# spacejam/tla-rust

Hardware: AMD Instinct MI355X
Metric: distinct states/sec, raft.tla (3 servers) (higher is better)
Workload: dtype u64

## Files before the change

### tla_rust_amd/csrc/engine.hip

```cpp
#include <hip/hip_runtime.h>
#include <hipcub/hipcub.hpp>

#include <algorithm>
#include <chrono>
#include <memory>
#include <type_traits>
#include <string>
#include <vector>

#include "spec_registry.h"
#include "hip_owned.h"

namespace mc {

#ifndef MC_TU
#define MC_TU -1
#endif
}
extern "C" void mc_set_error_internal(const char *msg);
namespace mc {
static void set_error(const std::string &s) { mc_set_error_internal(s.c_str()); }

#define HIP_TRY(expr)                                                                              \
    do {                                                                                           \
// ... 21 lines not shown
    double progress_interval = 1.0;
    std::chrono::steady_clock::time_point progress_last;
    bool stop_requested = false;
    void report_progress(uint32_t levels, uint64_t generated, uint64_t distinct, uint64_t queue) {
        if (!progress_fn) return;
        const auto now = std::chrono::steady_clock::now();
        if (std::chrono::duration<double>(now - progress_last).count() < progress_interval) return;
        progress_last = now;
        progress_fn(progress_user, levels, generated, distinct, queue);
    }
    virtual ~EngineBase() = default;
    virtual int run(mc_result *out) = 0;
    virtual int step(uint32_t levels, mc_result *out) = 0;
    virtual int trace(uint8_t *states_out, int32_t *actions_out, size_t *n_inout) = 0;
    virtual int kernel_stats(mc_kernel_stats *out) = 0;
    virtual int read_states(uint64_t first, uint64_t count, uint8_t *out) = 0;
    virtual int debug_reexpand(unsigned extra_flags, double *ms) = 0;
    virtual int debug_phases(uint64_t *out48, int reset) = 0;
    virtual int debug_flags(uint32_t set, uint32_t clear) = 0;
    virtual int checkpoint(const char *path) = 0;
    virtual int restore(const char *path) = 0;
    virtual int shard_begin() = 0;
    virtual int shard_begin_replicated(uint64_t min_frontier, uint64_t max_distinct, uint64_t max_levels, uint64_t *levels_out, uint32_t *nlevels) = 0;
    virtual int shard_level_size(uint64_t *n) = 0;
    virtual int shard_set_stream(void *hip_stream, int enable) = 0;
    virtual int shard_expand_launch(unsigned slot, uint64_t first, uint64_t count, uint64_t send_cap) = 0;
    virtual int shard_expand_finish(unsigned slot, uint64_t *send_fp, uint64_t send_cap, uint64_t *send_counts) = 0;
    virtual int shard_probe(const uint64_t *recv_fp, uint64_t n, uint8_t *answers) = 0;
    virtual int shard_expand_pack(unsigned slot, uint64_t *send_fp, uint64_t cap) = 0;
    virtual int shard_probe_pack(const uint64_t *recv_fp, uint64_t cap, uint8_t *answers) = 0;
    virtual int shard_keep_pack(unsigned slot, const uint8_t *answers_back, uint64_t cap) = 0;
    virtual int shard_wait_keep(unsigned slot) = 0;
    virtual int shard_materialise(unsigned slot, const uint8_t *answers_back, uint8_t *send_states, uint64_t send_cap, uint64_t *send_counts) = 0;
    virtual int shard_ingest(const uint8_t *recv_states, uint64_t n) = 0;
    virtual int shard_keep(unsigned slot, const uint8_t *answers_back, uint64_t *n_new) = 0;
    virtual int shard_end_level(uint64_t *new_local) = 0;
    virtual int shard_counters(uint64_t *generated, uint64_t *distinct_local, int32_t *verdict) = 0;
    virtual int shard_check_frontier() = 0;
    virtual int shard_materialise_parents(unsigned slot, uint64_t *send_parents) = 0;
    virtual int shard_ingest_parents(const uint64_t *recv_parents, uint64_t n, unsigned src_rank) = 0;
    virtual int shard_violation(int32_t *found, uint64_t *idx, uint32_t *slot, int32_t *verdict, int32_t *invariant) = 0;
    virtual int shard_fetch(uint64_t idx, uint8_t *state_out, uint32_t *parent_rank, uint64_t *parent_idx, uint32_t *parent_slot) = 0;
    virtual int shard_info(void **main_stream, uint64_t *chunk_states, int32_t *traced) = 0;
    virtual int shard_note_levels(const uint64_t *levels, uint32_t n, int32_t verdict) = 0;
    virtual int shard_resume(uint64_t *levels_out, uint32_t *nlevels) = 0;
    virtual int shard_checkpoint(const char *path) = 0;
    virtual int shard_restore(const char *path) = 0;
    virtual size_t state_bytes() const = 0;
    virtual int simulate(const mc_sim_opts *opts, mc_sim_result *out) = 0;
    virtual int coverage(mc_action_coverage *out, size_t *n_inout) = 0;
    virtual int graph(mc_graph_info *out) = 0;
    virtual int graph_read(uint64_t first, uint64_t count, uint64_t *offsets_out, uint32_t *dst_out, int32_t *action_out, size_t *nedges_inout) = 0;
    virtual int scc(mc_scc_info *out) = 0;
    virtual int scc_read(uint64_t first, uint64_t count, uint32_t *scc_out) = 0;
    virtual int liveness(uint64_t weak_fair_mask, mc_live_info *out) = 0;
    virtual int liveness_trace(uint32_t *prefix_out, size_t *nprefix_inout, uint32_t *cycle_out, size_t *ncycle_inout) = 0;
};

static uint64_t round_pow2(uint64_t v) {
    uint64_t p = 1;
    while (p < v) p <<= 1;
    return p;
}

struct KTimer {
    std::vector<Event> pool;
    struct Pending { int which; size_t e0, e1; uint64_t units; };
    std::vector<Pending> pending;
    size_t used = 0;
    bool enabled = false;
    hipEvent_t get() {
        if (used == pool.size()) pool.emplace_back(hipEventDefault);
        return pool[used++].get();
    }
    void resolve(mc_kernel_stat *stats ) {
        for (auto &p : pending) {
            float ms = 0;
            hipEventElapsedTime(&ms, pool[p.e0].get(), pool[p.e1].get());
            stats[p.which].launches++;
            stats[p.which].ms_total += ms;
            stats[p.which].units += p.units;
        }
        pending.clear();
        used = 0;
    }
};

template <class S, class = void>
struct HasExport : std::false_type {};
template <class S>
struct HasExport<S, decltype((void)S::EXPORT_WORDS)> : std::true_type {};
template <class S, class = void>
struct PackedRows : std::false_type {};
template <class S>
struct PackedRows<S, decltype((void)S::PACKED_ROWS)> : std::integral_constant<bool, S::PACKED_ROWS> {};

static_assert((unsigned)SIM_VK_INVARIANT == VK_INVARIANT && (unsigned)SIM_VK_ASSERT == VK_ASSERT && (unsigned)SIM_VK_DEADLOCK == VK_DEADLOCK, "one verdict_of_kind");
static int32_t verdict_of_kind(unsigned kind) {
    return kind == VK_INVARIANT ? MC_V_INVARIANT : kind == VK_ASSERT ? MC_V_ASSERT : kind == VK_DEADLOCK ? MC_V_DEADLOCK : MC_V_SPECERR;
}
struct Viol {
    unsigned kind, slot;
    int32_t verdict, invariant;
    explicit Viol(unsigned long long key)
        : kind((unsigned)(key & 7u)), slot((unsigned)(key >> 8 & 0xffffu)), verdict(verdict_of_kind(kind)), invariant(kind == VK_INVARIANT ? (int32_t)(key >> 3 & 31u) : -1) {}
    bool extra_state() const { return kind == VK_INVARIANT && slot < SLOT_PARENT; }
};

struct CkIdent {
    char magic[8];
    uint32_t spec_id, nparams;
    int64_t params[16];
    uint32_t words, has_trace;
};
struct CkHeader {
    CkIdent id;
    uint64_t distinct, generated, cells, lo, hi, nlevels;
};
struct ShCkHeader {
    CkIdent id;
    uint32_t rank, world;
    uint64_t table_cap, lo, hi, next, dup, nlevels;
};
struct ShCkCounters {
    uint64_t arena_next, viol_key, via_list;
    uint64_t generated[NSHARD], cells[NSHARD];
    uint32_t error, pad;
};
static_assert(sizeof(CkIdent) == 152 && offsetof(CkIdent, spec_id) == 8 && offsetof(CkIdent, params) == 16 && offsetof(CkIdent, words) == 144 && offsetof(CkIdent, has_trace) == 148, "checkpoint identity");
static_assert(sizeof(CkHeader) == 200 && offsetof(CkHeader, distinct) == 152 && offsetof(CkHeader, generated) == 160 && offsetof(CkHeader, cells) == 168 &&
              offsetof(CkHeader, lo) == 176 && offsetof(CkHeader, hi) == 184 && offsetof(CkHeader, nlevels) == 192, "TLAMCCK1 header");
static_assert(sizeof(ShCkHeader) == 208 && offsetof(ShCkHeader, rank) == 152 && offsetof(ShCkHeader, world) == 156 && offsetof(ShCkHeader, table_cap) == 160 &&
              offsetof(ShCkHeader, lo) == 168 && offsetof(ShCkHeader, hi) == 176 && offsetof(ShCkHeader, next) == 184 && offsetof(ShCkHeader, dup) == 192 &&
              offsetof(ShCkHeader, nlevels) == 200, "TLAMCSK2 header");
static_assert(NSHARD == 8 && sizeof(ShCkCounters) == 160 && offsetof(ShCkCounters, generated) == 24 && offsetof(ShCkCounters, cells) == 88 && offsetof(ShCkCounters, error) == 152, "TLAMCSK2 counters");
struct CkFormat { const char *magic, *writer, *reader, *not_ours, *other_program; };
static constexpr CkFormat CK_FUSED{"TLAMCCK1", "checkpoint", "restore", "not a checkpoint file",
                                   "the checkpoint was written by another compiled program (algorithm, constants, invariants or constraints differ)"};
static constexpr CkFormat CK_RANK{"TLAMCSK2", "mc_shard_checkpoint", "mc_shard_restore", "not a per-rank checkpoint file (of this library version)",
                                  "the checkpoint was written by another compiled program"};
struct CkPart { void *p; size_t bytes; };
struct FileCloser { FILE *f; ~FileCloser() { if (f) fclose(f); } };

template <class S>
struct Engine : EngineBase {
    using Params = typename S::Params;
    int W = 1;
    unsigned max_slots = 1;
    Params prm;
    mc_spec_desc desc;
    mc_config cfg;
    Stream stream, stream2;
    Stream stream_b;
    Event ev_level, ev_e[2], ev_m[2];
    DevBuf<uint64_t> d_arena, d_table, d_cand, d_inittmp;
    DevBuf<uint32_t> d_newlist, d_parent;
    DevBuf<uint64_t> d_newfp;
    DevBuf<uint16_t> d_nsl, d_pslot;
    DevBuf<uint8_t> d_prank;
    DevBuf<DevCounters> d_ctr;
    PinnedBuf<DevCounters> h_ctr;
    DevBuf<LevelCtl> d_lc;
    PinnedBuf<LevelCtl> h_lc;
    uint64_t table_cap = 0, arena_cap = 0, chunk = 0, row_stride = 0, seg_cap = 0;
    bool seen_sparse = false, use_matrix = false;
    bool no_slices = getenv("TLAMC_NOSLICE") != nullptr;
    double inwave_growth_limit = getenv("TLAMC_INWAVE_GROWTH") ? atof(getenv("TLAMC_INWAVE_GROWTH")) : 10.0;
    KTimer timer;
    mc_kernel_stat kstat[3];
    struct Fused {
        bool have_run = false, have_viol = false;
        unsigned long long last_viol = ~0ull;
        std::vector<uint64_t> level_start;
        uint64_t last_distinct = 0, last_generated = 0, cells = 0, inwave = 0;
        uint64_t stop_frontier = 0, lo = 0, hi = 0;
        bool mat_inwave_level = false;
        uint64_t mat_list_hint = 0;
    } fr;
    struct HandOver {
        bool pending = false, in_place = false;
        uint64_t distinct = 0, generated = 0, cells = 0, lo = 0;
        std::vector<uint64_t> level_start;
    } ck;
    struct ShSlot {
        DevBuf<uint64_t> rt_fp;
        DevBuf<uint32_t> rt_src, pend_src;
        DevBuf<PaddedCounter> rt_cur;
        uint64_t rt_subcap = 0, pend_total = 0, chunk_base = 0, count = 0, ncols = 0;
        BlockPlan plan;
        uint64_t moved = 0;
        OwnerOffsets pend_off;
        bool launched = false, keep_pending = false;
    };
    struct Shard {
        uint64_t lo = 0, hi = 0, next = 0;
        uint64_t dup = 0;
        ShSlot sl[2];
        DevBuf<uint32_t> d_new_src, d_incl;
        DevBuf<unsigned long long> d_ends;
        PinnedBuf<unsigned long long> h_ends;
        PinnedBuf<PaddedCounter> h_cur;
        DevBuf<char> d_scan_tmp;
        hipStream_t ext_stream = nullptr;
        bool ext_side = false;
        Event ev_slot[2], ev_keep[2], ev_ans;
        Event ev_append;
        Event ev_exp[2];
        Event ev_mat[2];
        std::vector<uint64_t> levels;
        bool ck_ok = false, resume = false;
        std::unique_ptr<mc_result> prefix_res{new mc_result()};
    } sh;
    struct Sim {
        DevBuf<uint64_t> buf[2];
        DevBuf<uint32_t> wst;
        DevBuf<SimCounters> ctr;
        std::vector<uint64_t> trace_rows;
        std::vector<int32_t> trace_acts;
        size_t trace_n = 0;
    } sim;
    struct Cov {
        bool on = false;
        int nbins = 0;
        DevBuf<unsigned long long> bins;
        std::vector<uint64_t> host;
        uint64_t init_generated = 0;
    } cov;
    struct Graph {
        bool built = false;
        DevBuf<uint64_t> offsets;
        DevBuf<uint32_t> dst;
        DevBuf<int16_t> act;
        mc_graph_info info{};
        struct Live {
            bool scc_built = false, checked = false;
            DevBuf<uint64_t> toff;
            DevBuf<uint32_t> tsrc;
            DevBuf<uint32_t> scc;
            DevBuf<uint32_t> size;
            DevBuf<int8_t> proc;
            DevBuf<unsigned long long> taken, disabled;
            DevBuf<unsigned> done;
            mc_scc_info sinfo{};
            mc_live_info linfo{};
            uint64_t fair = 0;
            void release() {
                scc_built = checked = false;
                toff.reset(); tsrc.reset(); scc.reset(); size.reset(); proc.reset(); taken.reset(); disabled.reset(); done.reset();
            }
        } lv;
        void release() { built = false; offsets.reset(); dst.reset(); act.reset(); lv.release(); }
    } gr;

    unsigned slices_for(uint64_t ncols, bool blind) const {
        if (!WantsSlices<S>::value || S::FIX_SLOTS != 0 || UsesFamilies<S>::value || pairs_only() || use_matrix || max_slots < 16 || no_slices) return 1;
        const uint64_t waves = (ncols + 63) / 64;
        uint64_t sg = blind ? 32 : (16384 + waves - 1) / waves;
        if (sg > 32) sg = 32;
        if (sg > max_slots / 4) sg = max_slots / 4;
        return sg < 1 ? 1u : (unsigned)sg;
    }
    uint64_t seen_arg() const { return seen_sparse ? ((table_cap / MC_SPARSE_SLOTS) | SEEN_SPARSE) : table_cap / 8; }
    unsigned nranks() const { return cfg.shard_count > 1 ? cfg.shard_count : 1; }

    int alloc() {
        W = S::words(prm);
        max_slots = (unsigned)S::max_slots(prm);
        use_matrix = (cfg.flags & MC_F_MATRIX) != 0;
        HIP_TRY(hipSetDevice(cfg.device));
        HIP_TRY(stream.create());
        {
            const char *pe = getenv("TLAMC_PRIO");
            int lo_p = 0, hi_p = 0;
            hipDeviceGetStreamPriorityRange(&lo_p, &hi_p);
            if (pe && *pe == '1') HIP_TRY(stream2.create(hi_p));
            else if (pe && *pe == '2') HIP_TRY(stream2.create(lo_p));
            else HIP_TRY(stream2.create());
        }
        for (int i = 0; i < 2; i++) { HIP_TRY(ev_e[i].create()); HIP_TRY(ev_m[i].create()); }
        {
            const char *es = getenv("TLAMC_EXPAND_STREAMS");
            if (es && *es == '2') {
                HIP_TRY(stream_b.create());
                HIP_TRY(ev_level.create());
            }
        }
        table_cap = cfg.table_capacity ? cfg.table_capacity : (1ull << 24);
        table_cap = (table_cap + 63) / 64 * 64;
        if (table_cap / 8 > 0xffffffffull) { set_error("table_capacity: at most 2^35 - 8 slots per device"); return MC_EBADCFG; }
        arena_cap = cfg.arena_capacity ? cfg.arena_capacity : (1ull << 22);
        arena_cap = (arena_cap + 63) & ~63ull;
        if (arena_cap >= (1ull << 32) - 1) { set_error("arena_capacity must be < 2^32 states"); return MC_EBADCFG; }
        static const double sparse_ratio = getenv("TLAMC_SPARSE_RATIO") && atof(getenv("TLAMC_SPARSE_RATIO")) >= 1.25 ? atof(getenv("TLAMC_SPARSE_RATIO")) : 3.0;
        seen_sparse = (double)table_cap >= sparse_ratio * (double)arena_cap && table_cap / MC_SPARSE_SLOTS <= 0xffffffffull && !getenv("TLAMC_DENSE_TABLE");
        chunk = cfg.chunk_states ? cfg.chunk_states : (1ull << 18);
        chunk = (chunk + 255) & ~255ull;
        if (chunk > (1ull << 24) - 256) chunk = (1ull << 24) - 256;
        if (max_slots > 255) { set_error("spec has more than 255 action slots per state"); return MC_EBADCFG; }
        row_stride = chunk + 256;
        HIP_TRY(d_arena.alloc(arena_cap * W));
        HIP_TRY(d_table.alloc(table_cap));
        HIP_TRY(d_cand.alloc((size_t)(use_matrix ? max_slots : 1) * row_stride));
        seg_cap = (row_stride / NSHARD + 256) * max_slots;
        seg_cap += seg_cap / 64 + 65;
        HIP_TRY(d_newlist.alloc((size_t)2 * NSHARD * seg_cap));
        if (HasKnownFp<S>::value && !use_matrix) HIP_TRY(d_newfp.alloc((size_t)2 * NSHARD * seg_cap));
        {
            const uint64_t ni = S::num_init(prm);
            HIP_TRY(d_inittmp.alloc((size_t)(ni < chunk ? ni : chunk) * W));
        }
        HIP_TRY(d_nsl.alloc(row_stride));
        if (cfg.flags & MC_F_TRACE) {
            HIP_TRY(d_parent.alloc(arena_cap));
            HIP_TRY(d_pslot.alloc(arena_cap));
            if (cfg.shard_count > 1) {
                HIP_TRY(d_prank.alloc(arena_cap));
                HIP_TRY(hipMemset(d_prank, 0xff, arena_cap));
            }
        }
        HIP_TRY(d_ctr.alloc(1));
        HIP_TRY(h_ctr.alloc(1));
        HIP_TRY(d_lc.alloc(1));
        HIP_TRY(h_lc.alloc(1));
        timer.enabled = (cfg.flags & MC_F_TIMING) != 0;
        if (cfg.flags & MC_F_COVERAGE) {
            cov.nbins = CovAction<S>::nbins(prm);
            if (cov.nbins > COV_MAX_BINS) { set_error("MC_F_COVERAGE: the model has more actions than the coverage histogram has bins (" + std::to_string(COV_MAX_BINS - 1) + ")"); return MC_EBADCFG; }
            HIP_TRY(cov.bins.alloc((size_t)2 * cov.nbins));
            HIP_TRY(hipMemset(cov.bins, 0, (size_t)2 * cov.nbins * sizeof(unsigned long long)));
            cov.host.assign((size_t)2 * cov.nbins, 0);
            cov.on = true;
        }
        return MC_OK;
    }

    void cov_generated(uint64_t lo, uint64_t hi) {
        for (uint64_t c0 = lo; c0 < hi;) {
            const uint64_t base = c0 & ~63ull;
            const uint64_t c1 = base + chunk < hi ? base + chunk : hi;
            const uint64_t ncols = ((c1 - base) + 63) & ~63ull;
            hipLaunchKernelGGL(k_coverage_generated<S>, dim3((unsigned)((ncols + 255) / 256)), dim3(256), 0, stream, prm, (const uint64_t *)d_arena,
                               c0, c1, ncols, cov.bins.p, cov.nbins);
            c0 = c1;
        }
    }
    void cov_distinct(uint64_t lo, uint64_t hi) {
        for (uint64_t c0 = lo; c0 < hi; c0 += chunk) {
            const uint64_t c1 = c0 + chunk < hi ? c0 + chunk : hi;
            hipLaunchKernelGGL(k_coverage_distinct<S>, dim3((unsigned)((c1 - c0 + 255) / 256)), dim3(256), 0, stream, prm, (const uint64_t *)d_arena,
                               (const uint32_t *)d_parent, (const uint16_t *)d_pslot, c0, c1, cov.bins.p + cov.nbins, cov.nbins);
        }
    }
    int cov_begin(uint64_t expanded, uint64_t stored) {
        HIP_TRY(hipMemsetAsync(cov.bins, 0, (size_t)2 * cov.nbins * sizeof(unsigned long long), stream));
        cov.init_generated = S::num_init(prm);
        cov_generated(0, expanded);
        cov_distinct(0, stored);
        return MC_OK;
    }
    int cov_end() {
        HIP_TRY(hipMemcpyAsync(cov.host.data(), cov.bins, cov.host.size() * sizeof(uint64_t), hipMemcpyDeviceToHost, stream));
        HIP_TRY(hipStreamSynchronize(stream));
        cov.host[0] += cov.init_generated;
        return MC_OK;
    }
    int coverage(mc_action_coverage *out, size_t *n_inout) override {
        if (!cov.on) { set_error("mc_engine_coverage: the engine was created without MC_F_COVERAGE"); return MC_ESTATE; }
        size_t n = 1;
        for (int a = 0; a + 1 < cov.nbins; a++) n += CovAction<S>::listed(prm, a) ? 1 : 0;
        if (n > *n_inout || !out) { *n_inout = n; set_error("mc_engine_coverage: buffer too small"); return MC_EBADCFG; }
        size_t k = 0;
        for (int a = -1; a + 1 < cov.nbins; a++) {
            if (a >= 0 && !CovAction<S>::listed(prm, a)) continue;
            out[k].action = a;
            out[k].pad = 0;
            out[k].generated = cov.host[(size_t)a + 1];
            out[k].distinct = cov.host[(size_t)cov.nbins + a + 1];
            k++;
        }
        *n_inout = n;
        return MC_OK;
    }

    template <class T>
    int graph_alloc(DevBuf<T> &b, size_t count, const char *what, const char *call = "mc_engine_graph") {
        if (b.alloc(count ? count : 1) == hipSuccess) return MC_OK;
        (void)hipGetLastError();
        set_error(std::string(call) + ": cannot allocate " + std::to_string((unsigned long long)(count * sizeof(T))) + " bytes of device memory for " + what);
        return MC_EARENA;
    }
    template <class K, class... A>
    void graph_chunks(K kernel, uint64_t lo, uint64_t hi, A... args) {
        for (uint64_t c0 = lo; c0 < hi;) {
            const uint64_t base = c0 & ~63ull;
            const uint64_t c1 = base + chunk < hi ? base + chunk : hi;
            const uint64_t ncols = ((c1 - base) + 63) & ~63ull;
            hipLaunchKernelGGL(kernel, dim3((unsigned)((ncols + 255) / 256)), dim3(256), 0, stream, prm, (const uint64_t *)d_arena, c0, c1, ncols,
                               (const uint64_t *)d_table, seen_arg(), args...);
            c0 = c1;
        }
    }
    int graph(mc_graph_info *out) override {
        memset(out, 0, sizeof *out);
        if (cfg.shard_count > 1) { set_error("mc_engine_graph: not available for a sharded engine (shard_count > 1)"); return MC_EBADCFG; }
        if (!fr.have_run || ck.pending) {
            set_error("mc_engine_graph: needs a search of this engine that returned a result (mc_engine_run / mc_engine_step; not a simulation, "
                      "not a restored checkpoint that has not run yet: its seen-set is not built)");
            return MC_ESTATE;
        }
        gr.release();
        const uint64_t n = fr.last_distinct, expanded = fr.lo;
        if (n + 1 > 0x7fffffffull) { set_error("mc_engine_graph: at most 2^31 - 2 states (the scan's item count)"); return MC_EBADCFG; }
        HIP_TRY(hipSetDevice(cfg.device));
        const auto t0 = std::chrono::steady_clock::now();
        DevBuf<uint32_t> slot_index, degree;
        DevBuf<GraphCounters> d_gc;
        DevBuf<char> scan_tmp;
        int rc;
        if ((rc = graph_alloc(slot_index, table_cap, "the fingerprint -> state index"))) return rc;
        if ((rc = graph_alloc(degree, n + 1, "the out-degrees"))) return rc;
        if ((rc = graph_alloc(gr.offsets, n + 1, "the row offsets"))) { gr.release(); return rc; }
        if ((rc = graph_alloc(d_gc, 1, "the counters"))) { gr.release(); return rc; }
        const int built = graph_build(n, expanded, slot_index, degree, d_gc, scan_tmp);
        if (built) { gr.release(); return built; }
        gr.info.states = n;
        gr.info.expanded = expanded;
        gr.info.init_states = fr.level_start.size() > 1 ? fr.level_start[1] : n;
        gr.info.seconds = std::chrono::duration<double>(std::chrono::steady_clock::now() - t0).count();
        gr.built = true;
        *out = gr.info;
        return MC_OK;
    }
    int graph_build(uint64_t n, uint64_t expanded, DevBuf<uint32_t> &slot_index, DevBuf<uint32_t> &degree, DevBuf<GraphCounters> &d_gc, DevBuf<char> &scan_tmp) {
        GraphCounters gc;
        memset(&gc, 0, sizeof gc);
        gc.first_bad = ~0ull;
        HIP_TRY(hipMemcpyAsync(d_gc, &gc, sizeof gc, hipMemcpyHostToDevice, stream));
        HIP_TRY(hipMemsetAsync(slot_index, 0xff, table_cap * sizeof(uint32_t), stream));
        HIP_TRY(hipMemsetAsync(degree, 0, (n + 1) * sizeof(uint32_t), stream));
        if (n) hipLaunchKernelGGL(k_graph_index<S>, dim3((unsigned)((n + 255) / 256)), dim3(256), 0, stream, prm, (const uint64_t *)d_arena, n,
                                  (const uint64_t *)d_table, seen_arg(), slot_index.p, table_cap, d_gc.p);
        graph_chunks(k_graph_degree<S>, 0, expanded, degree.p, d_gc.p);
        HIP_TRY(hipGetLastError());
        hipcub::TransformInputIterator<uint64_t, GraphDegreeCast, const uint32_t *> in(degree.p, GraphDegreeCast());
        size_t need = 0;
        HIP_TRY(hipcub::DeviceScan::ExclusiveSum(nullptr, need, in, gr.offsets.p, (int)(n + 1), stream));
        if (int rc = graph_alloc(scan_tmp, need, "the scan")) return rc;
        HIP_TRY(hipcub::DeviceScan::ExclusiveSum(scan_tmp.p, need, in, gr.offsets.p, (int)(n + 1), stream));
        uint64_t edges = 0;
        HIP_TRY(hipMemcpyAsync(&edges, gr.offsets.p + n, sizeof edges, hipMemcpyDeviceToHost, stream));
        HIP_TRY(hipMemcpyAsync(&gc, d_gc, sizeof gc, hipMemcpyDeviceToHost, stream));
        HIP_TRY(hipStreamSynchronize(stream));
        if (int rc = graph_inconsistent(gc)) return rc;
        if (int rc = graph_alloc(gr.dst, edges, "the edges' successors")) return rc;
// ... 225 lines not shown
            const size_t L = level_of(cur);
            uint64_t row[2];
            HIP_TRY(hipMemcpy(row, lv.toff.p + cur, sizeof row, hipMemcpyDeviceToHost));
            std::vector<uint32_t> src((size_t)(row[1] - row[0]));
            if (!src.empty()) HIP_TRY(hipMemcpy(src.data(), lv.tsrc.p + row[0], src.size() * sizeof(uint32_t), hipMemcpyDeviceToHost));
            uint32_t best = ~0u;
            for (uint32_t u : src) if (u >= fr.level_start[L - 1] && u < fr.level_start[L] && u < best) best = u;
            if (best == ~0u) { set_error("mc_engine_liveness_trace: state " + std::to_string(cur) + " has no in-edge from the level before its own"); return MC_ESTATE; }
            prefix.push_back(best);
            cur = best;
        }
        std::reverse(prefix.begin(), prefix.end());
        std::vector<uint64_t> off((size_t)n + 1);
        std::vector<uint32_t> dst((size_t)edges), scc((size_t)n);
        std::vector<int8_t> proc((size_t)edges);
        HIP_TRY(hipMemcpy(off.data(), gr.offsets.p, off.size() * sizeof(uint64_t), hipMemcpyDeviceToHost));
        HIP_TRY(hipMemcpy(scc.data(), lv.scc.p, scc.size() * sizeof(uint32_t), hipMemcpyDeviceToHost));
        if (edges) {
            HIP_TRY(hipMemcpy(dst.data(), gr.dst.p, dst.size() * sizeof(uint32_t), hipMemcpyDeviceToHost));
            HIP_TRY(hipMemcpy(proc.data(), lv.proc.p, proc.size() * sizeof(int8_t), hipMemcpyDeviceToHost));
        }
        std::vector<uint32_t> members;
        for (uint64_t v = 0; v < n; ++v) if (scc[(size_t)v] == root) members.push_back((uint32_t)v);
        std::vector<uint32_t> par((size_t)n, ~0u);
        std::vector<uint32_t> cycle{root};
        auto go = [&](uint32_t to) {
            const uint32_t from = cycle.back();
            if (from == to) return true;
            for (uint32_t m : members) par[m] = ~0u;
            std::vector<uint32_t> q{from};
            par[from] = from;
            for (size_t h = 0; h < q.size() && par[to] == ~0u; ++h)
                for (uint64_t k = off[q[h]]; k < off[q[h] + 1]; ++k) {
                    const uint32_t d = dst[(size_t)k];
                    if (scc[d] == root && par[d] == ~0u) { par[d] = q[h]; q.push_back(d); }
                }
            if (par[to] == ~0u) return false;
            std::vector<uint32_t> path;
            for (uint32_t x = to; x != from; x = par[x]) path.push_back(x);
            cycle.insert(cycle.end(), path.rbegin(), path.rend());
            return true;
        };
        bool ok = true;
        for (int p = 0; p < 64 && ok; ++p) {
            if (!(lv.fair >> p & 1)) continue;
            bool found = false;
            for (size_t mi = 0; mi < members.size() && !found; ++mi) {
                const uint32_t u = members[mi];
                for (uint64_t k = off[u]; k < off[u + 1] && !found; ++k)
                    if (proc[(size_t)k] == p && live_real_step(p, u, dst[(size_t)k]) && scc[dst[(size_t)k]] == root) {
                        found = true;
                        ok = go(u);
                        cycle.push_back(dst[(size_t)k]);
                    }
            }
            for (size_t mi = 0; mi < members.size() && !found; ++mi) {
                const uint32_t u = members[mi];
                uint64_t en = 0, tk = 0;
                bool dn = false;
                live_state(u, dst.data() + off[u], proc.data() + off[u], off[u + 1] - off[u], scc.data(), &en, &tk, &dn);
                if (!(en >> p & 1)) { found = true; ok = go(u); }
            }
            if (!found) ok = false;
        }
        if (ok) ok = go(root);
        if (!ok) { set_error("mc_engine_liveness_trace: the chosen component is not fair or not connected (the arrays disagree with the verdict)"); return MC_ESTATE; }
        cycle.pop_back();
        if (prefix.size() > *nprefix_inout || cycle.size() > *ncycle_inout || !prefix_out || (!cycle.empty() && !cycle_out)) {
            *nprefix_inout = prefix.size();
            *ncycle_inout = cycle.size();
            set_error("mc_engine_liveness_trace: buffers too small (" + std::to_string(prefix.size()) + " + " + std::to_string(cycle.size()) + " states)");
            return MC_EBADCFG;
        }
        memcpy(prefix_out, prefix.data(), prefix.size() * sizeof(uint32_t));
        if (!cycle.empty()) memcpy(cycle_out, cycle.data(), cycle.size() * sizeof(uint32_t));
        *nprefix_inout = prefix.size();
        *ncycle_inout = cycle.size();
        return MC_OK;
    }

    template <class F>
    void timed(int which, uint64_t units, F &&launch, hipStream_t on = nullptr) {
        if (!timer.enabled) { launch(); return; }
        if (!on) on = stream;
        hipEvent_t a = timer.get(), b = timer.get();
        size_t ia = timer.used - 2, ib = timer.used - 1;
        hipEventRecord(a, on);
        launch();
        hipEventRecord(b, on);
        timer.pending.push_back({which, ia, ib, units});
    }

    int read_counters() {
        if (stream_b) HIP_TRY(hipStreamSynchronize(stream_b));
        HIP_TRY(hipStreamSynchronize(stream2));
        HIP_TRY(hipMemcpyAsync(h_ctr, d_ctr, sizeof(DevCounters), hipMemcpyDeviceToHost, stream));
        HIP_TRY(hipStreamSynchronize(stream));
        if (timer.enabled) timer.resolve(kstat);
        return MC_OK;
    }
    int check_dev_error() {
        if (h_ctr->error & DEV_EOVERFLOW) { set_error("packed-state capacity exceeded (raft messages / elections / allLogs slots, or a PlusCal sequence longer than its cells, or a recursive PlusCal procedure deeper than $TLAMC_PCAL_STACK frames)"); return MC_EOVERFLOW; }
        if (h_ctr->error & DEV_ETABLE) { set_error("seen-set full: raise table_capacity"); return MC_ETABLEFULL; }
        if (h_ctr->error & DEV_EROUTE) { set_error("sharded round: an exchange bucket is full (raise the fan-out allowance / send capacity)"); return MC_EROUTE; }
        if (h_ctr->error & DEV_EARENA) { set_error("state arena full: raise arena_capacity"); return MC_EARENA; }
        return MC_OK;
    }

    bool inwave_ok() const { return (UsesFamilies<S>::value || UsesPairs<S>::value) && !use_matrix && !(cfg.flags & (MC_F_NOFAMILY | MC_F_NOINWAVE)); }
    bool pairs_only() const { return UsesPairs<S>::value && inwave_ok(); }
    void set_inwave(RouteArgs &rt) const {
        if (!inwave_ok()) return;
        rt.arena_w = d_arena;
        rt.arena_cap = arena_cap;
        rt.parent = d_parent;
        rt.pslot = d_pslot;
    }
    static unsigned mat_grid(uint64_t ncols) {
        const unsigned bx = (unsigned)((ncols + 255) / 256);
        const unsigned gm = bx < 8 * 256 ? (bx + 7) / 8 : 256;
        return gm ? gm : 1u;
    }
    void finish_materialise(uint64_t chunk_base, uint64_t ncols, unsigned parity, hipStream_t expanded_on = nullptr) {
        if (pairs_only()) return;
        unsigned gm = mat_grid(ncols);
        if (fr.mat_inwave_level) {
            const uint64_t want = (fr.mat_list_hint * 4 + 255) / 256;
            const unsigned per_seg = (unsigned)((want + NSHARD - 1) / NSHARD);
            if (per_seg < gm) gm = per_seg ? per_seg : 1u;
        }
        hipEventRecord(ev_e[parity].get(), expanded_on ? expanded_on : stream.s);
        hipStreamWaitEvent(stream2, ev_e[parity].get(), 0);
        timed(2, 0, [&] {
            hipLaunchKernelGGL(k_materialise<S>, dim3(gm, NSHARD), dim3(256), 0, stream2, prm, d_arena, chunk_base, d_newlist,
                               seg_cap, arena_cap, d_parent, d_pslot, d_ctr, parity, (const LevelCtl *)nullptr, (const uint64_t *)d_newfp);
        }, stream2);
        hipLaunchKernelGGL(k_commit, dim3(1), dim3(1), 0, stream2, d_ctr, parity);
        hipEventRecord(ev_m[parity].get(), stream2);
        static const bool serial = getenv("TLAMC_SERIAL") != nullptr;
        if (serial) hipStreamSynchronize(stream2);
    }
    void enqueue_blind_level(uint64_t max_states) {
        const uint64_t ncols = max_states + 64;
        RouteArgs rt{};
        rt.lc = d_lc;
        rt.new_fp = d_newfp;
        set_inwave(rt);
        const unsigned sg = slices_for(ncols, true);
        const bool dl = sg > 1 && (cfg.flags & MC_F_DEADLOCK);
        if (dl) { rt.succ = d_nsl; hipMemsetAsync(d_nsl, 0, ncols * sizeof(uint16_t), stream); }
        const unsigned lflags = cfg.flags | ((cfg.flags & MC_F_PARK) ? MC_FI_PARK : 0u);
        timed(0, 0, [&] {
            launch_expand<S, false>(!(cfg.flags & MC_F_NOFAMILY), lflags, ncols, stream, sg, prm, (const uint64_t *)d_arena,
                                    (uint64_t)0, (uint64_t)0, ncols, d_table.p, seen_arg(), d_newlist.p, seg_cap, d_ctr.p, cfg.flags, rt, 0u);
            if (dl) hipLaunchKernelGGL(k_deadlock_slices, dim3((unsigned)((ncols + 255) / 256)), dim3(256), 0, stream, (const uint16_t *)d_nsl,
                                       (uint64_t)0, (uint64_t)0, ncols, (const LevelCtl *)d_lc, d_ctr);
        });
        if (!pairs_only()) timed(2, 0, [&] {
            hipLaunchKernelGGL(k_materialise<S>, dim3(32, NSHARD), dim3(256), 0, stream, prm, d_arena, (uint64_t)0, d_newlist, seg_cap,
                               arena_cap, d_parent, d_pslot, d_ctr, 0u, (const LevelCtl *)d_lc, (const uint64_t *)d_newfp);
        });
        hipLaunchKernelGGL(k_end_level, dim3(1), dim3(1), 0, stream, d_ctr, d_lc);
    }

    template <bool INIT>
    void finish_chunk(uint64_t chunk_base_or_first, uint64_t ncols, unsigned rows) {
        const unsigned bx = (unsigned)((ncols + 255) / 256);
        timed(1, ncols * rows, [&] {
            hipLaunchKernelGGL(k_insert, dim3(bx, rows), dim3(256), 0, stream, d_cand, row_stride, ncols, d_nsl, d_table,
                               seen_arg(), d_newlist, d_ctr);
        });
        const unsigned gm = bx < 2048 ? bx : 2048;
        timed(2, 0, [&] {
            if (INIT)
                hipLaunchKernelGGL(k_init_materialise<S>, dim3(gm), dim3(256), 0, stream, prm, d_arena, chunk_base_or_first,
                                   d_inittmp, d_newlist, arena_cap, d_parent, d_pslot, d_ctr);
            else
                hipLaunchKernelGGL(k_materialise<S>, dim3(gm, 1), dim3(256), 0, stream, prm, d_arena, chunk_base_or_first,
                                   d_newlist, seg_cap, arena_cap, d_parent, d_pslot, d_ctr, 0u, (const LevelCtl *)nullptr, (const uint64_t *)nullptr);
        });
        hipLaunchKernelGGL(k_commit, dim3(1), dim3(1), 0, stream, d_ctr, 0u);
    }

    int seed_init(unsigned rank, unsigned count, bool resuming, bool in_place, std::chrono::steady_clock::time_point *t0) {
        if (!in_place) HIP_TRY(hipMemsetAsync(d_table, 0, table_cap * sizeof(uint64_t), stream));
        HIP_TRY(hipMemsetAsync(d_ctr, 0, sizeof(DevCounters), stream));
        DevCounters init_c;
        memset(&init_c, 0, sizeof init_c);
        init_c.viol_key = ~0ull;
        if (resuming) {
            init_c.arena_next = ck.distinct;
            init_c.generated[0].v = ck.generated;
            init_c.cells[0].v = ck.cells;
        }
        HIP_TRY(hipMemcpyAsync(d_ctr, &init_c, sizeof init_c, hipMemcpyHostToDevice, stream));
        if (t0) {
            HIP_TRY(hipStreamSynchronize(stream));
            *t0 = std::chrono::steady_clock::now();
        }
        if (resuming && ck.distinct && !in_place)
            hipLaunchKernelGGL(k_reseed_table<S>, dim3((unsigned)((ck.distinct + 255) / 256)), dim3(256), 0, stream, prm,
                               (const uint64_t *)d_arena, ck.distinct, d_table, seen_arg(), d_ctr);
        const uint64_t ninit = resuming ? 0 : S::num_init(prm);
        for (uint64_t first = 0; first < ninit; first += chunk) {
            const uint64_t n = ninit - first < chunk ? ninit - first : chunk;
            const uint64_t ncols = (n + 63) & ~63ull;
            hipLaunchKernelGGL(k_init_cand<S>, dim3((unsigned)((ncols + 255) / 256)), dim3(256), 0, stream, prm, first, n,
                               d_inittmp, d_cand, ncols, d_nsl, d_ctr, rank, count);
            finish_chunk<true>(first, ncols, 1);
        }
        return MC_OK;
    }
    int close_level(uint64_t &lo, uint64_t &hi, uint64_t new_hi, uint32_t &level, mc_result *out) {
        lo = hi;
        hi = new_hi;
        if (hi > lo) {
            fr.level_start.push_back(lo);
            if (level < MC_MAX_LEVELS) out->level_distinct[level] = hi - lo;
            level++;
        }
        if (level >= MC_MAX_LEVELS) { set_error("too many BFS levels"); return MC_EBADCFG; }
        return MC_OK;
    }

    int run(mc_result *out) override {
        memset(out, 0, sizeof *out);
        out->violated_invariant = -1;
        memset(kstat, 0, sizeof kstat);
        fr.have_viol = false;
        sim.trace_n = 0;
        stop_requested = false;
        gr.release();
        fr.have_run = false;
        fr.level_start.clear();
        HIP_TRY(hipSetDevice(cfg.device));
        const bool resuming = ck.pending, in_place = ck.pending && ck.in_place;
        ck.pending = ck.in_place = false;
        std::chrono::steady_clock::time_point t0;
        int rc = seed_init(0u, 1u, resuming, in_place, &t0);
        if (rc) return rc;
        progress_last = t0;
        auto progress = [&](uint32_t lv, uint64_t lo_, uint64_t hi_) {
            if (!progress_fn) return;
            uint64_t g = 0;
            for (int t = 0; t < NSHARD; t++) g += h_ctr->generated[t].v;
            report_progress(lv, g, hi_, hi_ - lo_);
        };
        if (inwave_ok()) hipLaunchKernelGGL(k_set_alloc_mode, dim3(1), dim3(1), 0, stream, d_ctr, 1u);
        bool alloc_atomic = inwave_ok();
        uint64_t prev_frontier = ~0ull >> 12;
        if ((rc = read_counters())) return rc;
        if ((rc = check_dev_error())) return rc;
        uint64_t lo = 0, hi = h_ctr->arena_next;
        uint32_t level = 1;
        out->level_distinct[0] = hi;
        fr.level_start.push_back(0);
        if (cov.on && !in_place && (rc = cov_begin(resuming ? ck.lo : 0, hi))) return rc;
        if (resuming) {
            fr.level_start = ck.level_start;
            level = (uint32_t)fr.level_start.size();
            lo = ck.lo;
            for (uint32_t k = 0; k < level && k < MC_MAX_LEVELS; k++)
                out->level_distinct[k] = (k + 1 < level ? fr.level_start[k + 1] : hi) - fr.level_start[k];
        }
        int budget = 0;
        uint64_t via_seen = 0;
        const bool park_levels = (cfg.flags & MC_F_PARK) != 0;
        fr.mat_list_hint = ~0ull >> 8;
        fr.mat_inwave_level = false;
        static const int blind_log2 = getenv("TLAMC_BLIND_LOG2") ? atoi(getenv("TLAMC_BLIND_LOG2")) : 20;
        uint64_t blind_max = 1ull << (blind_log2 >= 10 && blind_log2 <= 23 && slices_for((1ull << 16) + 64, true) == 1 ? blind_log2 : 16);
        if (chunk < blind_max) blind_max = chunk;
        while (hi > lo) {
            if (h_ctr->viol_key != ~0ull) break;
            if (fr.stop_frontier && hi - lo >= fr.stop_frontier) break;
            if (cfg.max_levels && level >= cfg.max_levels) { budget = 1; break; }
            if (cfg.max_distinct && hi >= cfg.max_distinct) { budget = 1; break; }
            if (stop_requested) { budget = 1; break; }
            if (!use_matrix && !(cfg.flags & MC_F_NOBATCH) && hi - lo <= blind_max) {
                memset(h_lc, 0, sizeof(LevelCtl));
                h_lc->lo = lo;
                h_lc->hi = hi;
                h_lc->max_states = blind_max;
                h_lc->max_distinct = cfg.max_distinct;
                h_lc->levels_left = cfg.max_levels ? (unsigned)(cfg.max_levels - level) : 0u;
                HIP_TRY(hipMemcpyAsync(d_lc, h_lc, sizeof(LevelCtl), hipMemcpyHostToDevice, stream));
                HIP_TRY(hipStreamSynchronize(stream2));
                if (inwave_ok() && !alloc_atomic) {
                    hipLaunchKernelGGL(k_set_alloc_mode, dim3(1), dim3(1), 0, stream, d_ctr, 1u);
                    alloc_atomic = true;
                }
                for (int k = 0; k < BLIND_BATCH; k++) enqueue_blind_level(blind_max);
                HIP_TRY(hipMemcpyAsync(h_lc, d_lc, sizeof(LevelCtl), hipMemcpyDeviceToHost, stream));
                if ((rc = read_counters())) return rc;
                if ((rc = check_dev_error())) return rc;
                for (unsigned k = 0; k < h_lc->nlev; k++) {
                    kstat[0].units += hi - lo;
                    if (cov.on) { cov_generated(lo, hi); cov_distinct(hi, h_lc->level_hi[k]); }
                    if ((rc = close_level(lo, hi, h_lc->level_hi[k], level, out))) return rc;
                }
                progress(level, lo, hi);
                prev_frontier = hi > lo ? hi - lo : 1;
                continue;
            }
            const bool lvl_inwave = inwave_ok() && (pairs_only() || (double)(hi - lo) <= inwave_growth_limit * (double)prev_frontier);
            if (inwave_ok() && lvl_inwave != alloc_atomic) {
                hipLaunchKernelGGL(k_set_alloc_mode, dim3(1), dim3(1), 0, stream, d_ctr, lvl_inwave ? 1u : 0u);
                alloc_atomic = lvl_inwave;
            }
            prev_frontier = hi - lo;
            fr.mat_inwave_level = lvl_inwave;
            unsigned chunk_no = 0;
            const bool two_streams = stream_b && !use_matrix && hi - lo > chunk && !(slices_for(chunk, false) > 1 && (cfg.flags & MC_F_DEADLOCK));
            if (two_streams) {
                hipEventRecord(ev_level.get(), stream);
                hipStreamWaitEvent(stream_b, ev_level.get(), 0);
            }
            for (uint64_t c0 = lo; c0 < hi; ++chunk_no) {
                const unsigned parity = chunk_no & 1u;
                const uint64_t base = c0 & ~63ull;
                uint64_t c1 = base + chunk;
                if (c1 > hi) c1 = hi;
                const uint64_t ncols = ((c1 - base) + 63) & ~63ull;
                if (use_matrix) {
                    timed(0, c1 - c0, [&] {
                        hipLaunchKernelGGL(k_expand<S>, dim3((unsigned)((ncols + 255) / 256)), dim3(256), 0, stream, prm, d_arena,
                                           c0, c1, d_cand, row_stride, ncols, d_nsl, d_ctr, cfg.flags);
                    });
                    finish_chunk<false>(base, ncols, max_slots);
                } else {
                    hipStream_t es = two_streams && parity ? stream_b.s : stream.s;
                    if (chunk_no >= 2) hipStreamWaitEvent(es, ev_m[parity].get(), 0);
                    RouteArgs rt_new{};
                    rt_new.new_fp = d_newfp;
                    if (lvl_inwave) set_inwave(rt_new);
                    const unsigned sg = slices_for(ncols, false);
                    const bool dl = sg > 1 && (cfg.flags & MC_F_DEADLOCK);
                    if (dl) { rt_new.succ = d_nsl; hipMemsetAsync(d_nsl, 0, ncols * sizeof(uint16_t), es); }
                    const unsigned lflags = cfg.flags | (lvl_inwave && park_levels ? MC_FI_PARK : 0u);
                    timed(0, c1 - c0, [&] {
                        launch_expand<S, false>(!(cfg.flags & MC_F_NOFAMILY), lflags, ncols, es, sg, prm,
                                                (const uint64_t *)d_arena, c0, c1, ncols, d_table.p, seen_arg(), d_newlist.p, seg_cap, d_ctr.p,
                                                cfg.flags, rt_new, parity);
                        if (dl) hipLaunchKernelGGL(k_deadlock_slices, dim3((unsigned)((ncols + 255) / 256)), dim3(256), 0, es,
                                                   (const uint16_t *)d_nsl, c0, c1, ncols, (const LevelCtl *)nullptr, d_ctr);
                    }, es);
                    finish_materialise(base, ncols, parity, es);
                }
                c0 = c1;
            }
            if ((rc = read_counters())) return rc;
            if ((rc = check_dev_error())) return rc;
            {
                const uint64_t via = h_ctr->via_list - via_seen;
                via_seen = h_ctr->via_list;
                const double growth = hi > lo ? (double)(h_ctr->arena_next - hi) / (double)(hi - lo) : 1.0;
                fr.mat_list_hint = (uint64_t)((double)(via / (chunk_no ? chunk_no : 1u)) * (growth > 1.0 ? growth : 1.0)) + 1;
            }
            if (cov.on) { cov_generated(lo, hi); cov_distinct(hi, h_ctr->arena_next); }
            if ((rc = close_level(lo, hi, h_ctr->arena_next, level, out))) return rc;
            progress(level, lo, hi);
        }
        if (cov.on && (rc = cov_end())) return rc;
        if (hi > lo && h_ctr->viol_key == ~0ull && !fr.stop_frontier && (rc = check_frontier(lo, hi))) return rc;
        const auto t1 = std::chrono::steady_clock::now();
        out->seconds = std::chrono::duration<double>(t1 - t0).count();
        out->distinct = h_ctr->arena_next;
        fr.last_distinct = h_ctr->arena_next;
        kstat[2].units = h_ctr->arena_next;
        out->generated = 0;
        fr.cells = 0;
        for (int t = 0; t < NSHARD; t++) { out->generated += h_ctr->generated[t].v; fr.cells += h_ctr->cells[t].v; }
        fr.last_generated = out->generated;
        fr.inwave = inwave_ok() && h_ctr->arena_next >= h_ctr->via_list + (resuming ? ck.distinct : 0)
                           ? h_ctr->arena_next - h_ctr->via_list - (resuming ? ck.distinct : 0) : 0;
        fr.have_run = true;
        out->queue_left = hi - lo;
        out->depth = level;
        out->levels = level;
        fr.lo = lo;
        fr.hi = hi;
        if (h_ctr->viol_key != ~0ull) {
            fr.have_viol = true;
            fr.last_viol = h_ctr->viol_key;
            const Viol v(fr.last_viol);
            out->verdict = v.verdict;
            out->violated_invariant = v.invariant;
            std::vector<uint64_t> chain;
            if (build_chain(chain) == MC_OK) out->trace_len = (uint32_t)chain.size() + (v.extra_state() ? 1u : 0u);
        } else {
            out->verdict = budget ? MC_V_BUDGET : MC_V_OK;
        }
        return MC_OK;
    }

    int step(uint32_t levels, mc_result *out) override {
        if (!levels) return MC_EBADCFG;
        const uint64_t saved = cfg.max_levels;
        const bool cont = fr.have_run && !fr.have_viol && fr.hi > fr.lo && !ck.pending;
        if (cont) {
            ck.distinct = fr.last_distinct; ck.generated = fr.last_generated; ck.cells = fr.cells; ck.lo = fr.lo;
            ck.level_start = fr.level_start;
            ck.pending = ck.in_place = true;
            cfg.max_levels = (uint64_t)fr.level_start.size() + levels;
        } else if (ck.pending) {
            cfg.max_levels = (uint64_t)ck.level_start.size() + levels;
        } else {
            cfg.max_levels = levels;
        }
        const int rc = run(out);
        cfg.max_levels = saved;
        if (rc) ck.pending = ck.in_place = false;
        return rc;
    }
    bool ck_params_comparable() const { return desc.spec_id != MC_SPEC_PCAL; }
    void ck_fill_ident(CkIdent &id, const CkFormat &fmt) const {
        memcpy(id.magic, fmt.magic, 8);
        id.spec_id = desc.spec_id;
        id.nparams = ck_params_comparable() ? desc.nparams : 1;
        for (uint32_t i = 0; i < id.nparams && i < 16; i++) id.params[i] = desc.params[i];
        if (!ck_params_comparable()) id.params[0] = (int64_t)program_hash;
        id.words = (uint32_t)W;
        id.has_trace = d_parent ? 1u : 0u;
    }
    static int ck_fail(int code, const char *who, const std::string &msg) { set_error(std::string(who) + ": " + msg); return code; }
    int ck_check_ident(const CkIdent &id, const CkFormat &fmt) const {
        if (memcmp(id.magic, fmt.magic, 8) != 0) return ck_fail(MC_EPARSE, fmt.reader, fmt.not_ours);
        if (id.spec_id != desc.spec_id || id.words != (uint32_t)W) return ck_fail(MC_EBADCFG, fmt.reader, "the checkpoint belongs to another spec");
        if (ck_params_comparable() && (id.nparams != desc.nparams || memcmp(id.params, desc.params, sizeof(int64_t) * (id.nparams < 16 ? id.nparams : 16)) != 0))
            return ck_fail(MC_EBADCFG, fmt.reader, "the checkpoint was written with other constants / invariants");
        if (!ck_params_comparable() && (id.nparams != 1 || (uint64_t)id.params[0] != program_hash)) return ck_fail(MC_EBADCFG, fmt.reader, fmt.other_program);
        return MC_OK;
    }
    std::vector<CkPart> ck_sections(uint64_t n, bool per_rank) const {
        std::vector<CkPart> v{{d_arena.p, (size_t)((n + 63) >> 6) * (size_t)W * 64 * sizeof(uint64_t)}};
        if (d_parent) {
            v.push_back({d_parent.p, (size_t)n * sizeof(uint32_t)});
            v.push_back({d_pslot.p, (size_t)n * sizeof(uint16_t)});
        }
        if (per_rank && d_prank) v.push_back({d_prank.p, (size_t)n});
        if (per_rank) v.push_back({d_table.p, (size_t)table_cap * sizeof(uint64_t)});
        return v;
    }
    int ck_write(const CkFormat &fmt, const char *path, std::initializer_list<CkPart> host, const std::vector<CkPart> &dev) {
        FILE *f = fopen(path, "wb");
        if (!f) return ck_fail(MC_EBADCFG, fmt.writer, std::string("cannot write ") + path);
        FileCloser closer{f};
        int rc = MC_OK;
        for (const CkPart &h : host)
            if (!rc && fwrite(h.p, 1, h.bytes, f) != h.bytes) rc = ck_fail(MC_EBADCFG, fmt.writer, "short write");
        for (const CkPart &d : dev) {
            if (rc) break;
            std::vector<char> buf(d.bytes < (64u << 20) ? d.bytes : (64u << 20));
            for (size_t off = 0; off < d.bytes && !rc; off += buf.size()) {
                const size_t n = d.bytes - off < buf.size() ? d.bytes - off : buf.size();
                HIP_TRY(hipMemcpy(buf.data(), (const char *)d.p + off, n, hipMemcpyDeviceToHost));
                if (fwrite(buf.data(), 1, n, f) != n) rc = ck_fail(MC_EBADCFG, "checkpoint", "short write");
            }
        }
        closer.f = nullptr;
        if (fclose(f) != 0 && !rc) rc = ck_fail(MC_EBADCFG, fmt.writer, "close failed");
        return rc;
    }
    template <class H>
    int ck_read_header(const CkFormat &fmt, FILE *f, H &h) const {
        if (fread(&h, sizeof h, 1, f) != 1) return ck_fail(MC_EPARSE, fmt.reader, fmt.not_ours);
        return ck_check_ident(h.id, fmt);
    }
    static int ck_read_host(const CkFormat &fmt, FILE *f, std::initializer_list<CkPart> host) {
        for (const CkPart &h : host)
            if (fread(h.p, 1, h.bytes, f) != h.bytes) return ck_fail(MC_EPARSE, fmt.reader, "the checkpoint file is truncated");
        return MC_OK;
    }
    static int ck_read_sections(FILE *f, const std::vector<CkPart> &dev) {
        for (const CkPart &d : dev) {
            std::vector<char> buf(d.bytes < (64u << 20) ? d.bytes : (64u << 20));
            for (size_t off = 0; off < d.bytes; off += buf.size()) {
                const size_t n = d.bytes - off < buf.size() ? d.bytes - off : buf.size();
                if (fread(buf.data(), 1, n, f) != n) return ck_fail(MC_EPARSE, "restore", "the checkpoint file is truncated");
                HIP_TRY(hipMemcpy((char *)d.p + off, buf.data(), n, hipMemcpyHostToDevice));
            }
        }
        return MC_OK;
    }
    int checkpoint(const char *path) override {
        if (cfg.shard_count > 1) { set_error("checkpoint: not available for a sharded engine"); return MC_EBADCFG; }
        if (!fr.have_run || fr.have_viol) { set_error("checkpoint: needs a completed mc_engine_run that stopped on a budget (or finished) without a violation"); return MC_EBADCFG; }
        HIP_TRY(hipSetDevice(cfg.device));
        HIP_TRY(hipDeviceSynchronize());
        CkHeader h;
        memset(&h, 0, sizeof h);
        ck_fill_ident(h.id, CK_FUSED);
        h.distinct = fr.last_distinct; h.generated = fr.last_generated; h.cells = fr.cells;
        h.lo = fr.lo; h.hi = fr.hi; h.nlevels = fr.level_start.size();
        return ck_write(CK_FUSED, path, {{&h, sizeof h}, {fr.level_start.data(), fr.level_start.size() * sizeof(uint64_t)}}, ck_sections(fr.last_distinct, false));
    }
    int restore(const char *path) override {
        if (cfg.shard_count > 1) { set_error("restore: not available for a sharded engine"); return MC_EBADCFG; }
        gr.release();
        FileCloser f{fopen(path, "rb")};
        if (!f.f) return ck_fail(MC_EPARSE, "restore", std::string("cannot read ") + path);
        CkHeader h;
        int rc = ck_read_header(CK_FUSED, f.f, h);
        if (rc) return rc;
        if (h.distinct * 10 > table_cap * 9) return ck_fail(MC_ETABLEFULL, "restore", "table_capacity cannot hold the checkpoint's states (load > 0.9)");
        if (h.distinct > arena_cap) return ck_fail(MC_EARENA, "restore", "arena_capacity is smaller than the checkpoint");
        if (h.hi != h.distinct || h.lo > h.hi || h.nlevels == 0 || h.nlevels >= MC_MAX_LEVELS) return ck_fail(MC_EPARSE, "restore", "inconsistent header");
        if (d_parent && !h.id.has_trace) return ck_fail(MC_EBADCFG, "restore", "the checkpoint holds no parent pointers (written without MC_F_TRACE); run without MC_F_TRACE");
        ck.level_start.assign((size_t)h.nlevels, 0);
        if ((rc = ck_read_host(CK_FUSED, f.f, {{ck.level_start.data(), ck.level_start.size() * sizeof(uint64_t)}}))) return rc;
        bool ok = ck.level_start[0] == 0 && ck.level_start.back() < h.hi && (h.lo == h.hi || ck.level_start.back() == h.lo);
        for (size_t k = 1; k < ck.level_start.size() && ok; k++) ok = ck.level_start[k] > ck.level_start[k - 1];
        if (!ok) return ck_fail(MC_EPARSE, "restore", "inconsistent level table");
        HIP_TRY(hipSetDevice(cfg.device));
        if ((rc = ck_read_sections(f.f, ck_sections(h.distinct, false)))) return rc;
// ... 1170 lines not shown
```

Before: 4.162 billion.

## Use a small nursery hash table while clearing the main table asynchronously

Early BFS levels now insert into a small nursery seen-table (2^25 slots by default) while the large main table is zeroed on a separate low-priority stream. Once the frontier or distinct count outgrows the nursery, the engine waits for the clear, reseeds the main table from the arena and switches back to it. This aims to hide the cost of the full-table memset at search start behind the small early levels. The cost is a reseed kernel, extra memory, and tighter caps on batched levels while in the nursery.

```diff
diff --git a/profiles/nursery_trace.py b/profiles/nursery_trace.py
--- /dev/null
+++ b/profiles/nursery_trace.py
@@ -0,0 +1,40 @@
+import csv
+import json
+import statistics
+import sys
+
+
+def main(path):
+    rows = []
+    with open(path, newline="") as f:
+        for r in csv.DictReader(f):
+            rows.append((int(r["Start_Timestamp"]), int(r["End_Timestamp"]), r["Kernel_Name"]))
+    rows.sort()
+    inits = [i for i, r in enumerate(rows) if "k_init_cand" in r[2]]
+    out = {"clear_ms": [], "small_ms": [], "overlap_ms": []}
+    for n, i in enumerate(inits):
+        end = inits[n + 1] if n + 1 < len(inits) else len(rows)
+        prev_end = max((r[1] for r in rows[:i] if "mc::" in r[2]), default=0)
+        run = rows[i:end]
+        ex = [k for k, r in enumerate(run) if "k_expand" in r[2]]
+        large = next((run[k] for j, k in enumerate(ex)
+                      if not any("k_end_level" in r[2] for r in run[k:ex[j + 1] if j + 1 < len(ex) else len(run)])), None)
+        if large is None:
+            continue
+        fills = [r for r in rows if "fill" in r[2].lower() and prev_end <= r[0] < large[0]]
+        if not fills:
+            continue
+        clear = max(fills, key=lambda r: r[1] - r[0])
+        t_init = rows[i][0]
+        out["clear_ms"].append((clear[1] - clear[0]) / 1e6)
+        out["small_ms"].append((large[0] - t_init) / 1e6)
+        out["overlap_ms"].append(max(0, min(clear[1], large[0]) - max(clear[0], t_init)) / 1e6)
+    line = {"searches": len(out["clear_ms"])}
+    for k, v in out.items():
+        line[k + "_median"] = round(statistics.median(v), 4) if v else None
+        line[k] = [round(x, 4) for x in v]
+    print(json.dumps(line))
+
+
+if __name__ == "__main__":
+    main(sys.argv[1])
diff --git a/tla_rust_amd/csrc/engine.hip b/tla_rust_amd/csrc/engine.hip
--- a/tla_rust_amd/csrc/engine.hip
+++ b/tla_rust_amd/csrc/engine.hip
@@ -197,8 +197,9 @@
     mc_config cfg;
     Stream stream, stream2;
     Stream stream_b;
-    Event ev_level, ev_e[2], ev_m[2];
-    DevBuf<uint64_t> d_arena, d_table, d_cand, d_inittmp;
+    Stream stream_clear;
+    Event ev_level, ev_e[2], ev_m[2], ev_clear, ev_seed;
+    DevBuf<uint64_t> d_arena, d_table, d_nursery, d_cand, d_inittmp;
     DevBuf<uint32_t> d_newlist, d_parent;
     DevBuf<uint64_t> d_newfp;
     DevBuf<uint16_t> d_nsl, d_pslot;
@@ -209,6 +210,8 @@
     PinnedBuf<LevelCtl> h_lc;
     uint64_t table_cap = 0, arena_cap = 0, chunk = 0, row_stride = 0, seg_cap = 0;
     bool seen_sparse = false, use_matrix = false;
+    uint64_t nursery_cap = 0, nursery_max_distinct = 0, nursery_max_states = 0;
+    bool in_nursery = false, clear_pending = false;
     bool no_slices = getenv("TLAMC_NOSLICE") != nullptr;
     double inwave_growth_limit = getenv("TLAMC_INWAVE_GROWTH") ? atof(getenv("TLAMC_INWAVE_GROWTH")) : 10.0;
     KTimer timer;
@@ -306,7 +309,13 @@
         return sg < 1 ? 1u : (unsigned)sg;
     }
     uint64_t seen_arg() const { return seen_sparse ? ((table_cap / MC_SPARSE_SLOTS) | SEEN_SPARSE) : table_cap / 8; }
+    uint64_t *live_table() const { return in_nursery ? d_nursery.p : d_table.p; }
+    uint64_t live_seen_arg() const {
+        if (!in_nursery) return seen_arg();
+        return seen_sparse ? ((nursery_cap / MC_SPARSE_SLOTS) | SEEN_SPARSE) : nursery_cap / 8;
+    }
     unsigned nranks() const { return cfg.shard_count > 1 ? cfg.shard_count : 1; }
+    ~Engine() { if (clear_pending) hipStreamSynchronize(stream_clear); }
 
     int alloc() {
         W = S::words(prm);
@@ -345,6 +354,27 @@
         row_stride = chunk + 256;
         HIP_TRY(d_arena.alloc(arena_cap * W));
         HIP_TRY(d_table.alloc(table_cap));
+        {
+            static const int nursery_log2 = [] {
+                const char *e = getenv("TLAMC_NURSERY_LOG2");
+                const int v = e ? atoi(e) : 25;
+                return v == 0 || (v >= 10 && v <= 30) ? v : 25;
+            }();
+            if (nursery_log2 && cfg.shard_count <= 1 && !use_matrix && (2ull << nursery_log2) <= table_cap) {
+                const uint64_t cap = 1ull << nursery_log2;
+                nursery_max_distinct = cap / 8;
+                nursery_max_states = (cap / 2 - cap / 8) / (max_slots ? max_slots : 1u);
+                if (nursery_max_states) {
+                    int lo_p = 0, hi_p = 0;
+                    hipDeviceGetStreamPriorityRange(&lo_p, &hi_p);
+                    HIP_TRY(stream_clear.create(lo_p));
+                    HIP_TRY(ev_clear.create());
+                    HIP_TRY(ev_seed.create());
+                    HIP_TRY(d_nursery.alloc(cap));
+                    nursery_cap = cap;
+                }
+            }
+        }
         HIP_TRY(d_cand.alloc((size_t)(use_matrix ? max_slots : 1) * row_stride));
         seg_cap = (row_stride / NSHARD + 256) * max_slots;
         seg_cap += seg_cap / 64 + 65;
@@ -876,7 +906,7 @@
         const unsigned lflags = cfg.flags | ((cfg.flags & MC_F_PARK) ? MC_FI_PARK : 0u);
         timed(0, 0, [&] {
             launch_expand<S, false>(!(cfg.flags & MC_F_NOFAMILY), lflags, ncols, stream, sg, prm, (const uint64_t *)d_arena,
-                                    (uint64_t)0, (uint64_t)0, ncols, d_table.p, seen_arg(), d_newlist.p, seg_cap, d_ctr.p, cfg.flags, rt, 0u);
+                                    (uint64_t)0, (uint64_t)0, ncols, live_table(), live_seen_arg(), d_newlist.p, seg_cap, d_ctr.p, cfg.flags, rt, 0u);
             if (dl) hipLaunchKernelGGL(k_deadlock_slices, dim3((unsigned)((ncols + 255) / 256)), dim3(256), 0, stream, (const uint16_t *)d_nsl,
                                        (uint64_t)0, (uint64_t)0, ncols, (const LevelCtl *)d_lc, d_ctr);
         });
@@ -891,8 +921,8 @@
     void finish_chunk(uint64_t chunk_base_or_first, uint64_t ncols, unsigned rows) {
         const unsigned bx = (unsigned)((ncols + 255) / 256);
         timed(1, ncols * rows, [&] {
-            hipLaunchKernelGGL(k_insert, dim3(bx, rows), dim3(256), 0, stream, d_cand, row_stride, ncols, d_nsl, d_table,
-                               seen_arg(), d_newlist, d_ctr);
+            hipLaunchKernelGGL(k_insert, dim3(bx, rows), dim3(256), 0, stream, d_cand, row_stride, ncols, d_nsl, live_table(),
+                               live_seen_arg(), d_newlist, d_ctr);
         });
         const unsigned gm = bx < 2048 ? bx : 2048;
         timed(2, 0, [&] {
@@ -906,8 +936,34 @@
         hipLaunchKernelGGL(k_commit, dim3(1), dim3(1), 0, stream, d_ctr, 0u);
     }
 
+    int settle_clear() {
+        in_nursery = false;
+        if (clear_pending) HIP_TRY(hipStreamSynchronize(stream_clear));
+        clear_pending = false;
+        return MC_OK;
+    }
+    int leave_nursery(uint64_t stored) {
+        HIP_TRY(hipStreamWaitEvent(stream, ev_clear.get(), 0));
+        if (stored)
+            hipLaunchKernelGGL(k_reseed_table<S>, dim3((unsigned)((stored + 255) / 256)), dim3(256), 0, stream, prm,
+                               (const uint64_t *)d_arena, stored, d_table, seen_arg(), d_ctr);
+        in_nursery = false;
+        return MC_OK;
+    }
     int seed_init(unsigned rank, unsigned count, bool resuming, bool in_place, std::chrono::steady_clock::time_point *t0) {
-        if (!in_place) HIP_TRY(hipMemsetAsync(d_table, 0, table_cap * sizeof(uint64_t), stream));
+        int rc = settle_clear();
+        if (rc) return rc;
+        if (nursery_cap && t0 && !resuming && S::num_init(prm) <= nursery_max_distinct) {
+            HIP_TRY(hipMemsetAsync(d_nursery, 0, nursery_cap * sizeof(uint64_t), stream));
+            HIP_TRY(hipEventRecord(ev_seed.get(), stream));
+            HIP_TRY(hipStreamWaitEvent(stream_clear, ev_seed.get(), 0));
+            HIP_TRY(hipMemsetAsync(d_table, 0, table_cap * sizeof(uint64_t), stream_clear));
+            clear_pending = true;
+            HIP_TRY(hipEventRecord(ev_clear.get(), stream_clear));
+            in_nursery = true;
+        } else if (!in_place) {
+            HIP_TRY(hipMemsetAsync(d_table, 0, table_cap * sizeof(uint64_t), stream));
+        }
         HIP_TRY(hipMemsetAsync(d_ctr, 0, sizeof(DevCounters), stream));
         DevCounters init_c;
         memset(&init_c, 0, sizeof init_c);
@@ -1001,12 +1057,14 @@
             if (cfg.max_levels && level >= cfg.max_levels) { budget = 1; break; }
             if (cfg.max_distinct && hi >= cfg.max_distinct) { budget = 1; break; }
             if (stop_requested) { budget = 1; break; }
-            if (!use_matrix && !(cfg.flags & MC_F_NOBATCH) && hi - lo <= blind_max) {
+            const bool batched = !use_matrix && !(cfg.flags & MC_F_NOBATCH) && hi - lo <= blind_max;
+            if (in_nursery && !(batched && hi < nursery_max_distinct && hi - lo <= nursery_max_states) && (rc = leave_nursery(hi))) return rc;
+            if (batched) {
                 memset(h_lc, 0, sizeof(LevelCtl));
                 h_lc->lo = lo;
                 h_lc->hi = hi;
-                h_lc->max_states = blind_max;
-                h_lc->max_distinct = cfg.max_distinct;
+                h_lc->max_states = in_nursery && nursery_max_states < blind_max ? nursery_max_states : blind_max;
+                h_lc->max_distinct = in_nursery && (!cfg.max_distinct || nursery_max_distinct < cfg.max_distinct) ? nursery_max_distinct : cfg.max_distinct;
                 h_lc->levels_left = cfg.max_levels ? (unsigned)(cfg.max_levels - level) : 0u;
                 HIP_TRY(hipMemcpyAsync(d_lc, h_lc, sizeof(LevelCtl), hipMemcpyHostToDevice, stream));
                 HIP_TRY(hipStreamSynchronize(stream2));
@@ -1085,6 +1143,11 @@
             if ((rc = close_level(lo, hi, h_ctr->arena_next, level, out))) return rc;
             progress(level, lo, hi);
         }
+        if (in_nursery) {
+            if ((rc = leave_nursery(h_ctr->arena_next))) return rc;
+            if ((rc = read_counters())) return rc;
+            if ((rc = check_dev_error())) return rc;
+        }
         if (cov.on && (rc = cov_end())) return rc;
         if (hi > lo && h_ctr->viol_key == ~0ull && !fr.stop_frontier && (rc = check_frontier(lo, hi))) return rc;
         const auto t1 = std::chrono::steady_clock::now();
```

Result: no change. 4.163 billion, median of 2 (+0.0%).
